# RchalYang/torchrl

Hardware: AMD Instinct MI355X
Metric: env_steps_per_sec_ppo_2048env_halfcheetah_shape (higher is better)
Workload: dtype f32

## Files before the change

torchrl_amd/csrc/k_ppo.hip:

```cpp
#include <cstdlib>
#include "trl_common.h"
#include "trl_mlp.h"
#include "trl_head.h"
#include "trl_comm.h"

struct PpoDev {
  const float *obs, *acts, *advs, *rets, *old_values, *old_logp;
  const int64_t* row_idx;
  int rows_mb, N;
  const double* adv_raw;
  double n_global;
  const float *pf_params, *vf_params;
  float clip_para, entropy_coeff;
  int clipped_value_loss, tanh_action;
  int loss_mode;
  float* partial;
  double* scal_partial;
  int n_wg, n_pf, p_stride;
  int D, A;
};

template <int D, int H, int A> struct PpoShape {
  static_assert(H == 64 && D > 16 && D <= 32 && A <= 8, "instantiated for 16 < D <= 32, H == 64, A <= 8");
  static constexpr int P_PF = MlpFlat<D, H, A>::P_PF, P_VF = MlpFlat<D, H, 1>::P_VF;
  static constexpr int P_STRIDE = ((P_PF > P_VF ? P_PF : P_VF) + 63) & ~63;
};

#define WV_WAVES 4
#ifdef TRL_EXP_CLK
#define WCLK_DECL long long clk_prev = clock64(); float clk_acc[24]; for (int q_ = 0; q_ < 24; ++q_) clk_acc[q_] = 0.f;
#define WCLK(ph) { __builtin_amdgcn_sched_barrier(0); const long long c_ = clock64(); clk_acc[ph] += (float)(c_ - clk_prev); clk_prev = c_; __builtin_amdgcn_sched_barrier(0); }
#else
#define WCLK_DECL
#define WCLK(ph)
#endif
#define WV_THREADS (64 * WV_WAVES)
#define LDT 20
#define LDW 68

template <int D, int H, int A> struct WvShape {
  static_assert(H == 64 && (D == 17 || D == 32) && A <= 8, "instantiated for D == 17 / 32, H == 64, A <= 8");
  static constexpr int O_W2F = 0, O_W2B = H * LDW, O_B1 = 2 * H * LDW, O_B2 = O_B1 + H, O_SCR = O_B2 + H;
  static constexpr int O_H1 = 0, O_H2 = H * LDT, O_DZ2 = 2 * H * LDT, O_DO = 3 * H * LDT, WSCR = O_DO + 16 * LDT;
  static constexpr int P_STRIDE = PpoShape<D, H, A>::P_STRIDE;
  static constexpr int MAIN = O_SCR + WV_WAVES * WSCR;
  static constexpr int XS_W2 = 0, XS_W1 = 16, XS_W1B = 20, XS_W3 = D > 17 ? 24 : 20, XS_PF = XS_W3 + 4, XS_VF = XS_W3;
  static constexpr int XSC_PF = 3 * H + 32, XSC_VF = 4 * H + 16;
  static constexpr int XCH_PF = WV_WAVES * (XS_PF * 256 + XSC_PF), XCH_VF = WV_WAVES * (XS_VF * 256 + XSC_VF);
  static constexpr int XCH = XCH_PF > XCH_VF ? XCH_PF : XCH_VF;
  static constexpr int LDS_FLOATS = MAIN > XCH ? MAIN : XCH;
};

template <int D, int H, int A> struct WvShapeSD : WvShape<D, H, A> {
  static constexpr int P_PF_SD = H * D + H + H * H + H + 2 * A * H + 2 * A, P_VF = MlpFlat<D, H, 1>::P_VF;
  static constexpr int P_STRIDE = ((P_PF_SD > P_VF ? P_PF_SD : P_VF) + 63) & ~63;
};
template <int D, int H, int A, int HEAD> struct WvPick { using T = WvShape<D, H, A>; };
template <int D, int H, int A> struct WvPick<D, H, A, HEAD_SD> { using T = WvShapeSD<D, H, A>; };
#define SD_HALF_LOG_2PI_PLUS_HALF 1.4189385332046727f

__device__ __forceinline__ f32x4 lds4(const float* p) { return *reinterpret_cast<const f32x4*>(p); }
__device__ __forceinline__ float row_sum16(float v) {
  v += __builtin_bit_cast(float, __builtin_amdgcn_update_dpp(0, __builtin_bit_cast(int, v), 0x128, 0xF, 0xF, false));
  v += __builtin_bit_cast(float, __builtin_amdgcn_update_dpp(0, __builtin_bit_cast(int, v), 0x124, 0xF, 0xF, false));
  v += __builtin_bit_cast(float, __builtin_amdgcn_update_dpp(0, __builtin_bit_cast(int, v), 0x122, 0xF, 0xF, false));
  v += __builtin_bit_cast(float, __builtin_amdgcn_update_dpp(0, __builtin_bit_cast(int, v), 0x121, 0xF, 0xF, false));
  return v;
}

template <int D, int H, int A, int ACT, bool IS_PF, bool CONTIG, bool RT, int HEAD = HEAD_GAUSS>
__device__ void ppo_wave_pass(const PpoDev& a, float* lds, int wg_in_net, int n_wg_net) {
  using S = typename WvPick<D, H, A, HEAD>::T;
  constexpr bool WIDE = D > 17,
                 CAT = HEAD == HEAD_CAT, SD = HEAD == HEAD_SD,
                 SDP = SD && IS_PF;
  static_assert(!WIDE || RT, "the wide tile exists as a runtime-dims instantiation only");
  static_assert(!CAT || (IS_PF && RT), "the categorical head is a policy pass of the runtime-dims kernels");
  static_assert(!SD || RT, "the state-dependent-std head belongs to the runtime-dims kernels");
  constexpr int AS = CAT ? 1 : 0;
  const int Dr = RT ? a.D : D;
  const int O = IS_PF ? (RT ? a.A : A) : 1;
  const int OH = SDP ? 2 * O : O;
  const int F_W1 = 0, F_B1 = H * Dr, F_W2 = F_B1 + H, F_B2 = F_W2 + H * H, F_W3 = F_B2 + H, F_B3 = F_W3 + OH * H,
            F_LS = F_B3 + OH, F_END = (CAT || SDP) ? F_LS : F_LS + O;
  auto sd_has = [&](int o) -> bool { return (o & 7) < O; };
  auto sd_row = [&](int o) -> int { return o < 8 ? o : O + (o - 8); };
  const int PS = RT ? a.p_stride : S::P_STRIDE;
  const int tid = threadIdx.x, lane = tid & 63, wave = tid >> 6;
  const int j = lane & 15, g = lane >> 4, i = j;
  const float* gp = IS_PF ? a.pf_params : a.vf_params;
  WCLK_DECL
  float* W2F = lds + S::O_W2F;
  float* W2B = lds + S::O_W2B;
  float* scr = lds + S::O_SCR + wave * S::WSCR;
  float* H1S = scr + S::O_H1;
  float* H2S = scr + S::O_H2;
  float* DZ2S = scr + S::O_DZ2;
  float* DOS = scr + S::O_DO;

  const double adv_s1 = IS_PF ? a.adv_raw[0] : 0.0, adv_s2 = IS_PF ? a.adv_raw[1] : 0.0;
  const int B = a.rows_mb * a.N;
  const int n_tiles = (B + 15) / 16;
  const int tile_stride = n_wg_net * WV_WAVES;

  float xq[5], xtq[4], lq[6];
  float xq2[4], xtq2[4];
  int tile = wg_in_net * WV_WAVES + wave;
  const int tpr = a.N >> 4;
  int p1r = 0, p1c = 0, p2r = 0, p2c = 0, st_r = 0, st_c = 0;
  int64_t ridx1 = 0, ridx2 = 0;
  bool fv[4], fv2[4];
  const bool f16 = !WIDE && (!RT || Dr > 16), jv = !RT || i < Dr, jv2 = WIDE && 16 + i < Dr;
  const unsigned ox16 = (unsigned)(j * Dr + (f16 ? 16 : 0)) * 4u, os = (unsigned)j * 4u;
  unsigned oxq[4], oxt[4], oa_[4], oxq2[4], oxt2[4];
#pragma unroll
  for (int q = 0; q < 4; ++q) {
    fv[q] = !RT || 4 * g + q < Dr;
    fv2[q] = WIDE && 16 + 4 * g + q < Dr;
    oxq[q] = (unsigned)(j * Dr + (fv[q] ? 4 * g + q : 0)) * 4u;
    oxt[q] = (unsigned)((4 * g + q) * Dr + (jv ? i : 0)) * 4u;
    oxq2[q] = (unsigned)(j * Dr + (fv2[q] ? 16 + 4 * g + q : 0)) * 4u;
    oxt2[q] = (unsigned)((4 * g + q) * Dr + (jv2 ? 16 + i : 0)) * 4u;
    if constexpr (SDP) oa_[q] = (unsigned)(j * O + (4 * (g & 1) + q < O ? 4 * (g & 1) + q : 0)) * 4u;
    else oa_[q] = CAT ? (unsigned)j * 4u : (unsigned)(j * O + (4 * g + q < O ? 4 * g + q : 0)) * 4u;
  }
  auto ldb = [](const float* base, unsigned byte_off) -> float {
    return *reinterpret_cast<const float*>(reinterpret_cast<const char*>(base) + byte_off);
  };
  auto pos_advance = [&](int& r, int& c) { c += st_c; r += st_r; if (c >= tpr) { c -= tpr; ++r; } };
  auto load_ridx = [&](int r) -> int64_t {
    const int rr = r < a.rows_mb ? r : 0;
    return a.row_idx ? a.row_idx[rr] : (int64_t)rr;
  };
  auto fetch_contig = [&](int64_t ridx, int r, int c) {
    const int64_t cell0 = (r < a.rows_mb) ? ridx * a.N + 16 * c : 0;
    const float* ob = a.obs + cell0 * Dr;
#pragma unroll
    for (int q = 0; q < 4; ++q) xq[q] = ldb(ob, oxq[q]);
    xq[4] = ldb(ob, ox16);
#pragma unroll
    for (int q = 0; q < 4; ++q) xtq[q] = ldb(ob, oxt[q]);
    if constexpr (WIDE) {
#pragma unroll
      for (int q = 0; q < 4; ++q) { xq2[q] = ldb(ob, oxq2[q]); xtq2[q] = ldb(ob, oxt2[q]); }
    }
    if constexpr (IS_PF) {
      const float* ab = a.acts + cell0 * (CAT ? AS : O);
      if constexpr (CAT) { lq[0] = ldb(ab, oa_[0]); lq[1] = lq[2] = lq[3] = 0.0f; }
      else {
#pragma unroll
        for (int q = 0; q < 4; ++q) lq[q] = ldb(ab, oa_[q]);
      }
      lq[4] = ldb(a.advs + cell0, os);
      lq[5] = a.old_logp ? ldb(a.old_logp + cell0, os) : 0.0f;
    } else {
      lq[0] = lq[1] = lq[2] = lq[3] = 0.0f;
      lq[4] = ldb(a.rets + cell0, os);
      lq[5] = a.clipped_value_loss ? ldb(a.old_values + cell0, os) : 0.0f;
    }
  };
  auto row_of = [&](int smp, int& e) -> int { const int sm = smp < B ? smp : 0; const int r = sm / a.N; e = sm - r * a.N; return r; };
  auto fetch_inputs = [&](int64_t p, int s0) {
#pragma unroll
    for (int r = 0; r < 4; ++r) xq[r] = a.obs[p * Dr + (fv[r] ? 4 * g + r : 0)];
    xq[4] = a.obs[p * Dr + (f16 ? 16 : 0)];
#pragma unroll
    for (int q = 0; q < 4; ++q) {
      const int sj = 4 * g + q;
      const int64_t pr = __shfl(p, sj, 64);
      xtq[q] = a.obs[(s0 + sj < B ? pr : 0) * Dr + (jv ? i : 0)];
      if constexpr (WIDE) {
        xq2[q] = a.obs[p * Dr + (fv2[q] ? 16 + 4 * g + q : 0)];
        xtq2[q] = a.obs[(s0 + sj < B ? pr : 0) * Dr + (jv2 ? 16 + i : 0)];
      }
    }
    if constexpr (IS_PF) {
      if constexpr (CAT) { lq[0] = a.acts[p]; lq[1] = lq[2] = lq[3] = 0.0f; }
      else if constexpr (SDP) {
#pragma unroll
        for (int r = 0; r < 4; ++r) lq[r] = a.acts[p * O + (4 * (g & 1) + r < O ? 4 * (g & 1) + r : 0)];
      } else {
#pragma unroll
        for (int r = 0; r < 4; ++r) lq[r] = a.acts[p * O + (4 * g + r < O ? 4 * g + r : 0)];
      }
      lq[4] = a.advs[p]; lq[5] = a.old_logp ? a.old_logp[p] : 0.0f;
    } else {
      lq[0] = lq[1] = lq[2] = lq[3] = 0.0f;
      lq[4] = a.rets[p]; lq[5] = a.clipped_value_loss ? a.old_values[p] : 0.0f;
    }
  };
  int e_nn = 0;
  int64_t ridx_nn = 0;
  auto fetch_row = [&](int t) {
    const int r = row_of(t * 16 + j, e_nn);
    ridx_nn = a.row_idx ? a.row_idx[r] : (int64_t)r;
  };
  auto prefetch_next = [&](int nt) {
    if constexpr (CONTIG) {
      fetch_contig(ridx1, p1r, p1c);
      p1r = p2r; p1c = p2c; ridx1 = ridx2;
      pos_advance(p2r, p2c);
      ridx2 = load_ridx(p2r);
    } else {
      const int64_t pn = (nt * 16 + j < B) ? ridx_nn * a.N + e_nn : 0;
      fetch_inputs(pn, nt * 16);
      fetch_row(nt + tile_stride);
    }
  };
  if constexpr (CONTIG) {
    const int t0 = __builtin_amdgcn_readfirstlane(tile);
    const int ts = __builtin_amdgcn_readfirstlane(tile_stride);
    st_r = ts / tpr; st_c = ts - st_r * tpr;
    int r0 = t0 / tpr, c0 = t0 - (t0 / tpr) * tpr;
    fetch_contig(load_ridx(r0), r0, c0);
    p1r = r0; p1c = c0;
    pos_advance(p1r, p1c);
    ridx1 = load_ridx(p1r);
    p2r = p1r; p2c = p1c;
    pos_advance(p2r, p2c);
    ridx2 = load_ridx(p2r);
  } else {
    fetch_row(tile);
    const int64_t p0 = (tile * 16 + j < B) ? ridx_nn * a.N + e_nn : 0;
    fetch_inputs(p0, tile * 16);
    fetch_row(tile + tile_stride);
  }
  constexpr int NV = H * H / (4 * WV_THREADS);
  f32x4 wv[NV], wt[NV];
  const int tc = tid & 63, tq = tid >> 6;
  const float bias1 = tid < H ? gp[F_B1 + tid] : 0.0f, bias2 = tid < H ? gp[F_B2 + tid] : 0.0f;
  {
    static_assert(WV_THREADS == 256 && H == 64, "the transposed staging maps (column, 4 rows) onto 256 threads");
    const bool w2_al = !RT || ((reinterpret_cast<uintptr_t>(gp + F_W2) & 15) == 0);
#pragma unroll
    for (int t = 0; t < NV; ++t) {
      if (w2_al) wv[t] = *reinterpret_cast<const f32x4*>(gp + F_W2 + 4 * (tid + WV_THREADS * t));
      else {
#pragma unroll
        for (int x = 0; x < 4; ++x) wv[t][x] = gp[F_W2 + 4 * (tid + WV_THREADS * t) + x];
      }
    }
#pragma unroll
    for (int t = 0; t < NV; ++t)
#pragma unroll
      for (int x = 0; x < 4; ++x) wt[t][x] = gp[F_W2 + (4 * (tq + 4 * t) + x) * H + tc];
  }
  for (int e = lane; e < 16 * LDT; e += 64) DOS[e] = 0.0f;
  float w1[4][5], w3h[4][4], w3t[4][4];
  float w1b[4][4];
#pragma unroll
  for (int so = 0; so < 4; ++so) {
    const int row = 16 * so + i;
#pragma unroll
    for (int r = 0; r < 4; ++r) w1[so][r] = fv[r] ? gp[F_W1 + row * Dr + (fv[r] ? 4 * g + r : 0)] : 0.0f;
    w1[so][4] = (g == 0 && f16) ? gp[F_W1 + row * Dr + (f16 ? 16 : 0)] : 0.0f;
    if constexpr (WIDE) {
#pragma unroll
      for (int r = 0; r < 4; ++r) w1b[so][r] = fv2[r] ? gp[F_W1 + row * Dr + (fv2[r] ? 16 + 4 * g + r : 0)] : 0.0f;
    }
#pragma unroll
    for (int r = 0; r < 4; ++r) {
      if constexpr (SDP) {
        const int o = 4 * g + r;
        w3h[so][r] = sd_has(i) ? gp[F_W3 + (sd_has(i) ? sd_row(i) : 0) * H + 16 * so + 4 * g + r] : 0.0f;
        w3t[so][r] = sd_has(o) ? gp[F_W3 + (sd_has(o) ? sd_row(o) : 0) * H + row] : 0.0f;
      } else if constexpr (IS_PF) {
        w3h[so][r] = (i < O) ? gp[F_W3 + (i < O ? i : 0) * H + 16 * so + 4 * g + r] : 0.0f;
        const int o = 4 * g + r;
        w3t[so][r] = (o < O) ? gp[F_W3 + (o < O ? o : 0) * H + row] : 0.0f;
      } else {
        w3h[so][r] = gp[F_W3 + 16 * so + 4 * g + r];
        w3t[so][r] = 0.0f;
      }
    }
  }
  float lsv[4], ivv[4], b3v[4], lspass[4];
#pragma unroll
  for (int r = 0; r < 4; ++r) {
    const int o = 4 * g + r;
    const float raw = (IS_PF && !CAT && !SDP && o < O) ? gp[F_LS + (o < O ? o : 0)] : 0.0f;
    lsv[r] = fminf(fmaxf(raw, -20.0f), 2.0f);
    ivv[r] = __expf(-2.0f * lsv[r]);
    lspass[r] = (raw >= -20.0f && raw <= 2.0f) ? 1.0f : 0.0f;
    if constexpr (SDP) b3v[r] = sd_has(o) ? gp[F_B3 + (sd_has(o) ? sd_row(o) : 0)] : 0.0f;
    else b3v[r] = (o < O) ? gp[F_B3 + (o < O ? o : 0)] : 0.0f;
  }
  const float vb3 = IS_PF ? 0.0f : gp[F_B3];
#ifdef TRL_EXP_CLK
  WCLK(22)
  __builtin_amdgcn_s_waitcnt(0);
  WCLK(23)
#endif
#pragma unroll
  for (int t = 0; t < NV; ++t) {
    const int e = 4 * (tid + WV_THREADS * t), r = e / H, c = e - r * H;
    *reinterpret_cast<f32x4*>(W2F + r * LDW + c) = wv[t];
    *reinterpret_cast<f32x4*>(W2B + tc * LDW + 4 * (tq + 4 * t)) = wt[t];
  }
  if (tid < H) { lds[S::O_B1 + tid] = bias1; lds[S::O_B2 + tid] = bias2; }
  __syncthreads();

  const double ng = a.n_global;
  const double adv_mean = adv_s1 / ng;
  const double adv_var = (adv_s2 - adv_s1 * adv_s1 / ng) / (ng - 1.0);
  const float adv_mu = (float)adv_mean;
  const float adv_rstd = 1.0f / ((float)sqrt(fmax(adv_var, 0.0)) + 1e-5f);
  const float inv_b = (float)(1.0 / ng);

  f32x4 gW2[4][4], gW1[4], gW3[4];
  f32x4 gW1b[4];
  float gb1[4][4], gb2[4][4], gW1c[4][4];
  float db3[4], dls[4], stv[7];
  float ent_sum = 0.0f;
  float sdst[8] = {0.0f, 0.0f, -INFINITY, -INFINITY, 0.0f, 0.0f, -INFINITY, -INFINITY}, sd_cnt = 0.0f;
#pragma unroll
  for (int x = 0; x < 4; ++x) {
    gW1[x] = gW3[x] = gW1b[x] = f32x4{0.f, 0.f, 0.f, 0.f};
    db3[x] = dls[x] = 0.0f;
#pragma unroll
    for (int y = 0; y < 4; ++y) { gW2[x][y] = f32x4{0.f, 0.f, 0.f, 0.f}; gb1[x][y] = gb2[x][y] = gW1c[x][y] = 0.0f; }
  }
#pragma unroll
  for (int k = 0; k < 7; ++k) stv[k] = (k >= 2 && k <= 5) ? -INFINITY : 0.0f;

  WCLK(0)
  for (; tile < n_tiles; tile += tile_stride) {
    const int s = tile * 16 + j;
    const bool valid = CONTIG ? true : (s < B);
    float xb[5], xt[4], lin[6], xb2[4], xt2[4];
#pragma unroll
    for (int r = 0; r < 4; ++r) xb[r] = (valid && fv[r]) ? xq[r] : 0.0f;
    xb[4] = (valid && f16) ? xq[4] : 0.0f;
#pragma unroll
    for (int q = 0; q < 4; ++q) xt[q] = (jv && (CONTIG || tile * 16 + 4 * g + q < B)) ? xtq[q] : 0.0f;
    if constexpr (WIDE) {
#pragma unroll
      for (int q = 0; q < 4; ++q) {
        xb2[q] = (valid && fv2[q]) ? xq2[q] : 0.0f;
        xt2[q] = (jv2 && (CONTIG || tile * 16 + 4 * g + q < B)) ? xtq2[q] : 0.0f;
      }
    }
#pragma unroll
    for (int q = 0; q < 6; ++q) lin[q] = lq[q];
    const float x16 = xb[4];

#define PIN_DS() __builtin_amdgcn_sched_barrier(0x676)
    f32x4 h1[4], h2[4];
    f32x4 wq[4], bq;
#pragma unroll
    for (int so = 0; so < 4; ++so) h1[so] = lds4(lds + S::O_B1 + 16 * so + 4 * g);
#pragma unroll
    for (int sl = 0; sl < 4; ++sl) wq[sl] = lds4(W2F + i * LDW + 16 * sl + 4 * g);
    bq = lds4(lds + S::O_B2 + 4 * g);
    PIN_DS();
    WCLK(9)
#pragma unroll
    for (int q = 0; q < (WIDE ? 4 : 5); ++q)
#pragma unroll
      for (int so = 0; so < 4; ++so) h1[so] = mfma16(w1[so][q], xb[q], h1[so]);
    if constexpr (WIDE) {
#pragma unroll
      for (int q = 0; q < 4; ++q)
#pragma unroll
        for (int so = 0; so < 4; ++so) h1[so] = mfma16(w1b[so][q], xb2[q], h1[so]);
    }
    WCLK(10)
#pragma unroll
    for (int so = 0; so < 4; ++so)
#pragma unroll
      for (int r = 0; r < 4; ++r) {
        h1[so][r] = act_fn<ACT>(h1[so][r]);
        H1S[(16 * so + 4 * g + r) * LDT + j] = h1[so][r];
      }
    WCLK(1)
#pragma unroll
    for (int so = 0; so < 4; ++so) {
      f32x4 acc = bq;
      f32x4 wc[4];
#pragma unroll
      for (int sl = 0; sl < 4; ++sl) wc[sl] = wq[sl];
      if (so < 3) {
#pragma unroll
        for (int sl = 0; sl < 4; ++sl) wq[sl] = lds4(W2F + (16 * (so + 1) + i) * LDW + 16 * sl + 4 * g);
        bq = lds4(lds + S::O_B2 + 16 * (so + 1) + 4 * g);
        PIN_DS();
      }
#pragma unroll
      for (int sl = 0; sl < 4; ++sl)
#pragma unroll
        for (int r = 0; r < 4; ++r) acc = mfma16(wc[sl][r], h1[sl][r], acc);
      WCLK(11)
#pragma unroll
      for (int r = 0; r < 4; ++r) h2[so][r] = act_fn<ACT>(acc[r]);
      WCLK(12)
    }

    prefetch_next(tile + tile_stride);
    WCLK(2)
    f32x4 dz2[4];
    f32x4 wb[4];
    if constexpr (IS_PF) {
#pragma unroll
      for (int so = 0; so < 4; ++so)
#pragma unroll
        for (int r = 0; r < 4; ++r) H2S[(16 * so + 4 * g + r) * LDT + j] = h2[so][r];
      f32x4 oa = f32x4{b3v[0], b3v[1], b3v[2], b3v[3]}, ob = f32x4{0.f, 0.f, 0.f, 0.f};
#pragma unroll
      for (int sl = 0; sl < 4; sl += 2)
#pragma unroll
        for (int r = 0; r < 4; ++r) { oa = mfma16(w3h[sl][r], h2[sl][r], oa); ob = mfma16(w3h[sl + 1][r], h2[sl + 1][r], ob); }
      WCLK(14)
      float zc[4], lp = 0.0f;
      float pk[4], lpk[4], ent = 0.0f;
      int ai = 0;
      if constexpr (CAT) {
        float lg[4], ek[4], m = -INFINITY;
#pragma unroll
        for (int r = 0; r < 4; ++r) {
          lg[r] = oa[r] + ob[r];
          m = (4 * g + r < O) ? fmaxf(m, lg[r]) : m;
        }
        m = fmaxf(m, __shfl_xor(m, 16, 64));
        m = g < 2 ? m : 0.0f;
#pragma unroll
        for (int r = 0; r < 4; ++r) ek[r] = (4 * g + r < O) ? expf(lg[r] - m) : 0.0f;
        const float c_own = ((ek[0] + ek[1]) + ek[2]) + ek[3];
        const float c_lo = __shfl_xor(c_own, 16, 64);
        float Ssum = g == 1 ? (((c_lo + ek[0]) + ek[1]) + ek[2]) + ek[3] : c_own;
        const float S_hi = __shfl_xor(Ssum, 16, 64);
        Ssum = g == 0 ? S_hi : (g == 1 ? Ssum : 1.0f);
        const float logS = logf(Ssum);
        ai = min(max((int)lin[0], 0), O - 1);
#pragma unroll
        for (int r = 0; r < 4; ++r) {
          const bool has = 4 * g + r < O;
          lpk[r] = has ? (lg[r] - m) - logS : 0.0f;
          pk[r] = ek[r] / Ssum;
          lp += (has && 4 * g + r == ai) ? lpk[r] : 0.0f;
          ent -= pk[r] * lpk[r];
        }
        lp += __shfl_xor(lp, 16, 64);
        ent += __shfl_xor(ent, 16, 64);
      } else if constexpr (SDP) {
#pragma unroll
        for (int r = 0; r < 4; ++r) {
          const bool has = 4 * (g & 1) + r < O;
          const float mine = oa[r] + ob[r], oth = __shfl_xor(mine, 32, 64);
          const float mean = g < 2 ? mine : oth, raw = g < 2 ? oth : mine;
          lsv[r] = fminf(fmaxf(raw, -20.0f), 2.0f);
          ivv[r] = __expf(-2.0f * lsv[r]);
          lspass[r] = (raw >= -20.0f && raw <= 2.0f) ? 1.0f : 0.0f;
          const float t = gauss_logp_term((valid && has) ? lin[r] : 0.0f, has ? mean : 0.0f, ivv[r], lsv[r], a.tanh_action, zc[r]);
          lp += has ? t : 0.0f;
          ent += has ? SD_HALF_LOG_2PI_PLUS_HALF + lsv[r] : 0.0f;
          zc[r] = has ? zc[r] : 0.0f;
        }
        lp += __shfl_xor(lp, 16, 64);
        ent += __shfl_xor(ent, 16, 64);
      } else {
#pragma unroll
      for (int r = 0; r < 4; ++r) {
        const bool has = 4 * g + r < O;
        const float t = gauss_logp_term((valid && has) ? lin[r] : 0.0f, has ? oa[r] + ob[r] : 0.0f, ivv[r], lsv[r],
                                        a.tanh_action, zc[r]);
        lp += has ? t : 0.0f;
        zc[r] = has ? zc[r] : 0.0f;
      }
      WCLK(18)
      lp += __shfl_xor(lp, 16, 64);
      }
      WCLK(19)
      const float advn = valid ? (lin[4] - adv_mu) * adv_rstd : 0.0f;
      float ratio, s1, s2, g_lp;
      if (a.loss_mode == TRL_LOSS_A2C) {
        ratio = 1.0f;
        s1 = s2 = lp * advn;
        g_lp = (valid && (SDP || g < 2)) ? -advn * inv_b : 0.0f;
      } else {
        ratio = __expf(lp - lin[5]);
        s1 = ratio * advn;
        s2 = fminf(fmaxf(ratio, 1.0f - a.clip_para), 1.0f + a.clip_para) * advn;
        g_lp = (valid && (SDP || g < 2) && s1 <= s2) ? -advn * ratio * inv_b : 0.0f;
      }
      WCLK(20)
      float dout[4];
      if constexpr (CAT) {
        const float ce = a.entropy_coeff * inv_b;
#pragma unroll
        for (int r = 0; r < 4; ++r) {
          const bool own = valid && g < 2 && 4 * g + r < O;
          dout[r] = own ? g_lp * ((4 * g + r == ai ? 1.0f : 0.0f) - pk[r]) + ce * pk[r] * (lpk[r] + ent) : 0.0f;
          db3[r] += dout[r];
          if (g < 2) DOS[(4 * g + r) * LDT + j] = dout[r];
        }
        if (valid && g == 0) ent_sum += ent;
      } else if constexpr (SDP) {
        const float ce = a.entropy_coeff * inv_b;
#pragma unroll
        for (int r = 0; r < 4; ++r) {
          const bool own = valid && 4 * (g & 1) + r < O;
          const float dm = g_lp * zc[r] * ivv[r], dr = lspass[r] * (g_lp * (zc[r] * zc[r] * ivv[r] - 1.0f) - ce);
          dout[r] = own ? (g < 2 ? dm : dr) : 0.0f;
          db3[r] += dout[r];
          DOS[(4 * g + r) * LDT + j] = dout[r];
          if (own && g < 2) {
            const float x = lsv[r], ex = expf(x);
            sdst[0] += x; sdst[1] = fmaf(x, x, sdst[1]); sdst[2] = fmaxf(sdst[2], x); sdst[3] = fmaxf(sdst[3], -x);
            sdst[4] += ex; sdst[5] = fmaf(ex, ex, sdst[5]); sdst[6] = fmaxf(sdst[6], ex); sdst[7] = fmaxf(sdst[7], -ex);
          }
        }
        if (valid && g == 0) { ent_sum += ent; sd_cnt += 1.0f; }
      } else {
#pragma unroll
      for (int r = 0; r < 4; ++r) {
        const bool own = valid && g < 2 && 4 * g + r < O;
        dout[r] = own ? g_lp * zc[r] * ivv[r] : 0.0f;
        db3[r] += dout[r];
        dls[r] += own ? lspass[r] * (g_lp * (zc[r] * zc[r] * ivv[r] - 1.0f) - a.entropy_coeff * inv_b) : 0.0f;
        if (g < 2) DOS[(4 * g + r) * LDT + j] = dout[r];
      }
      }
      WCLK(21)
      if (valid && g == 0) {
        stv[0] += lp; stv[1] = fmaf(lp, lp, stv[1]); stv[6] -= fminf(s1, s2);
        stv[2] = fmaxf(stv[2], lp); stv[3] = fmaxf(stv[3], -lp);
        stv[4] = fmaxf(stv[4], ratio); stv[5] = fmaxf(stv[5], -ratio);
      }
      WCLK(15)
      const f32x4 da = lds4(DOS + i * LDT + 4 * g);
      f32x4 hb3[4];
#pragma unroll
      for (int so = 0; so < 4; ++so) hb3[so] = lds4(H2S + (16 * so + j) * LDT + 4 * g);
#pragma unroll
      for (int so = 0; so < 4; ++so) wb[so] = lds4(W2B + (16 * so + i) * LDW + 4 * g);
      PIN_DS();
#pragma unroll
      for (int so = 0; so < 4; ++so) dz2[so] = f32x4{0.f, 0.f, 0.f, 0.f};
#pragma unroll
      for (int r = 0; r < 4; ++r)
#pragma unroll
        for (int so = 0; so < 4; ++so) dz2[so] = mfma16(w3t[so][r], dout[r], dz2[so]);
#pragma unroll
      for (int so = 0; so < 4; ++so)
#pragma unroll
        for (int q = 0; q < 4; ++q) gW3[so] = mfma16(da[q], hb3[so][q], gW3[so]);
      WCLK(16)
    } else {
#pragma unroll
      for (int so = 0; so < 4; ++so) wb[so] = lds4(W2B + (16 * so + i) * LDW + 4 * g);
      PIN_DS();
      float v = 0.0f;
#pragma unroll
      for (int so = 0; so < 4; ++so)
#pragma unroll
        for (int r = 0; r < 4; ++r) v = fmaf(w3h[so][r], h2[so][r], v);
      v += __shfl_xor(v, 16, 64);
      v += __shfl_xor(v, 32, 64);
      v += vb3;
      const float R = lin[4];
      float dv, l;
      if (a.clipped_value_loss) {
        const float vo = lin[5];
        const float dc = v - vo;
        const float vc = vo + fminf(fmaxf(dc, -a.clip_para), a.clip_para);
        const float l1 = (v - R) * (v - R), l2 = (vc - R) * (vc - R);
        const float wa = l1 > l2 ? 1.0f : (l1 == l2 ? 0.5f : 0.0f), wb_ = 1.0f - wa;
        const float pass = (dc >= -a.clip_para && dc <= a.clip_para) ? 1.0f : 0.0f;
        l = 0.5f * fmaxf(l1, l2);
        dv = inv_b * (wa * (v - R) + wb_ * pass * (vc - R));
      } else {
        l = (v - R) * (v - R);
        dv = 2.0f * (v - R) * inv_b;
      }
      dv = valid ? dv : 0.0f;
      if (valid && g == 0) {
        stv[6] += l; db3[0] += dv;
        stv[0] += v; stv[1] = fmaf(v, v, stv[1]); stv[2] = fmaxf(stv[2], v); stv[3] = fmaxf(stv[3], -v);
      }
#pragma unroll
      for (int so = 0; so < 4; ++so)
#pragma unroll
        for (int r = 0; r < 4; ++r) {
          dz2[so][r] = dv * w3h[so][r];
          gW3[so][r] = fmaf(dv, h2[so][r], gW3[so][r]);
        }
    }
#pragma unroll
    for (int so = 0; so < 4; ++so)
#pragma unroll
      for (int r = 0; r < 4; ++r) {
        dz2[so][r] *= act_grad<ACT>(h2[so][r]);
        gb2[so][r] += dz2[so][r];
        DZ2S[(16 * so + 4 * g + r) * LDT + j] = dz2[so][r];
      }

    WCLK(3)
    f32x4 dz1[4];
    f32x4 hb[4], za2;
#pragma unroll
    for (int so = 0; so < 4; ++so) dz1[so] = f32x4{0.f, 0.f, 0.f, 0.f};
#pragma unroll
    for (int sl = 0; sl < 4; ++sl) {
      f32x4 w[4];
// ... 1128 lines not shown
```

Measured before the change: 101.6 million.

## Stage non-W2 parameters through a coalesced LDS image before per-lane gathers

The prologue of the PPO wave pass now loads all parameters except W2 (W1, biases, W3, b3, log-std) cooperatively and coalesced into registers, then writes them to a new LDS image region. Per-lane W1/W3/b3/log-std values are then read from LDS instead of scattered global loads, and the predicate masking is applied after the reads. Input prefetch is moved after the weight loads and fenced with sched_barriers to control issue order. This costs extra LDS per workgroup, which may reduce occupancy, and adds an extra LDS round trip in the prologue.

```diff
diff --git a/torchrl_amd/csrc/k_ppo.hip b/torchrl_amd/csrc/k_ppo.hip
--- a/torchrl_amd/csrc/k_ppo.hip
+++ b/torchrl_amd/csrc/k_ppo.hip
@@ -48,12 +48,18 @@
   static constexpr int XSC_PF = 3 * H + 32, XSC_VF = 4 * H + 16;
   static constexpr int XCH_PF = WV_WAVES * (XS_PF * 256 + XSC_PF), XCH_VF = WV_WAVES * (XS_VF * 256 + XSC_VF);
   static constexpr int XCH = XCH_PF > XCH_VF ? XCH_PF : XCH_VF;
-  static constexpr int LDS_FLOATS = MAIN > XCH ? MAIN : XCH;
+  static constexpr int O_IMG = MAIN > XCH ? MAIN : XCH;
+  static constexpr int IMG_HEAD = 8 * H + 16;
+  static constexpr int IMG = (H * D + 2 * H + IMG_HEAD + WV_THREADS - 1) / WV_THREADS * WV_THREADS;
+  static constexpr int LDS_FLOATS = O_IMG + IMG;
 };
 
 template <int D, int H, int A> struct WvShapeSD : WvShape<D, H, A> {
   static constexpr int P_PF_SD = H * D + H + H * H + H + 2 * A * H + 2 * A, P_VF = MlpFlat<D, H, 1>::P_VF;
   static constexpr int P_STRIDE = ((P_PF_SD > P_VF ? P_PF_SD : P_VF) + 63) & ~63;
+  static constexpr int IMG_HEAD = 16 * H + 16;
+  static constexpr int IMG = (H * D + 2 * H + IMG_HEAD + WV_THREADS - 1) / WV_THREADS * WV_THREADS;
+  static constexpr int LDS_FLOATS = WvShape<D, H, A>::O_IMG + IMG;
 };
 template <int D, int H, int A, int HEAD> struct WvPick { using T = WvShape<D, H, A>; };
 template <int D, int H, int A> struct WvPick<D, H, A, HEAD_SD> { using T = WvShapeSD<D, H, A>; };
@@ -207,12 +213,48 @@
       fetch_row(nt + tile_stride);
     }
   };
+  int r0 = 0, c0 = 0;
+  int64_t ridx0 = 0;
   if constexpr (CONTIG) {
     const int t0 = __builtin_amdgcn_readfirstlane(tile);
     const int ts = __builtin_amdgcn_readfirstlane(tile_stride);
     st_r = ts / tpr; st_c = ts - st_r * tpr;
-    int r0 = t0 / tpr, c0 = t0 - (t0 / tpr) * tpr;
-    fetch_contig(load_ridx(r0), r0, c0);
+    r0 = t0 / tpr; c0 = t0 - (t0 / tpr) * tpr;
+    ridx0 = load_ridx(r0);
+  } else {
+    fetch_row(tile);
+  }
+  __builtin_amdgcn_sched_barrier(0);
+  constexpr int NV = H * H / (4 * WV_THREADS);
+  f32x4 wv[NV], wt[NV];
+  const int tc = tid & 63, tq = tid >> 6;
+  {
+    static_assert(WV_THREADS == 256 && H == 64, "the transposed staging maps (column, 4 rows) onto 256 threads");
+    const bool w2_al = !RT || ((reinterpret_cast<uintptr_t>(gp + F_W2) & 15) == 0);
+#pragma unroll
+    for (int t = 0; t < NV; ++t) {
+      if (w2_al) wv[t] = *reinterpret_cast<const f32x4*>(gp + F_W2 + 4 * (tid + WV_THREADS * t));
+      else {
+#pragma unroll
+        for (int x = 0; x < 4; ++x) wv[t][x] = gp[F_W2 + 4 * (tid + WV_THREADS * t) + x];
+      }
+    }
+#pragma unroll
+    for (int t = 0; t < NV; ++t)
+#pragma unroll
+      for (int x = 0; x < 4; ++x) wt[t][x] = gp[F_W2 + (4 * (tq + 4 * t) + x) * H + tc];
+  }
+  constexpr int NI = S::IMG / WV_THREADS;
+  const int n_img = F_W2 + (F_END - F_B2);
+  float im[NI];
+#pragma unroll
+  for (int k = 0; k < NI; ++k) {
+    const int e = tid + WV_THREADS * k, ec = e < n_img ? e : n_img - 1;
+    im[k] = gp[ec < F_W2 ? ec : ec + H * H];
+  }
+  __builtin_amdgcn_sched_barrier(0);
+  if constexpr (CONTIG) {
+    fetch_contig(ridx0, r0, c0);
     p1r = r0; p1c = c0;
     pos_advance(p1r, p1c);
     ridx1 = load_ridx(p1r);
@@ -220,85 +262,100 @@
     pos_advance(p2r, p2c);
     ridx2 = load_ridx(p2r);
   } else {
-    fetch_row(tile);
     const int64_t p0 = (tile * 16 + j < B) ? ridx_nn * a.N + e_nn : 0;
     fetch_inputs(p0, tile * 16);
     fetch_row(tile + tile_stride);
   }
-  constexpr int NV = H * H / (4 * WV_THREADS);
-  f32x4 wv[NV], wt[NV];
-  const int tc = tid & 63, tq = tid >> 6;
-  const float bias1 = tid < H ? gp[F_B1 + tid] : 0.0f, bias2 = tid < H ? gp[F_B2 + tid] : 0.0f;
-  {
-    static_assert(WV_THREADS == 256 && H == 64, "the transposed staging maps (column, 4 rows) onto 256 threads");
-    const bool w2_al = !RT || ((reinterpret_cast<uintptr_t>(gp + F_W2) & 15) == 0);
-#pragma unroll
-    for (int t = 0; t < NV; ++t) {
-      if (w2_al) wv[t] = *reinterpret_cast<const f32x4*>(gp + F_W2 + 4 * (tid + WV_THREADS * t));
-      else {
-#pragma unroll
-        for (int x = 0; x < 4; ++x) wv[t][x] = gp[F_W2 + 4 * (tid + WV_THREADS * t) + x];
-      }
-    }
-#pragma unroll
-    for (int t = 0; t < NV; ++t)
-#pragma unroll
-      for (int x = 0; x < 4; ++x) wt[t][x] = gp[F_W2 + (4 * (tq + 4 * t) + x) * H + tc];
-  }
-  for (int e = lane; e < 16 * LDT; e += 64) DOS[e] = 0.0f;
-  float w1[4][5], w3h[4][4], w3t[4][4];
-  float w1b[4][4];
-#pragma unroll
-  for (int so = 0; so < 4; ++so) {
-    const int row = 16 * so + i;
-#pragma unroll
-    for (int r = 0; r < 4; ++r) w1[so][r] = fv[r] ? gp[F_W1 + row * Dr + (fv[r] ? 4 * g + r : 0)] : 0.0f;
-    w1[so][4] = (g == 0 && f16) ? gp[F_W1 + row * Dr + (f16 ? 16 : 0)] : 0.0f;
-    if constexpr (WIDE) {
-#pragma unroll
-      for (int r = 0; r < 4; ++r) w1b[so][r] = fv2[r] ? gp[F_W1 + row * Dr + (fv2[r] ? 16 + 4 * g + r : 0)] : 0.0f;
-    }
-#pragma unroll
-    for (int r = 0; r < 4; ++r) {
-      if constexpr (SDP) {
-        const int o = 4 * g + r;
-        w3h[so][r] = sd_has(i) ? gp[F_W3 + (sd_has(i) ? sd_row(i) : 0) * H + 16 * so + 4 * g + r] : 0.0f;
-        w3t[so][r] = sd_has(o) ? gp[F_W3 + (sd_has(o) ? sd_row(o) : 0) * H + row] : 0.0f;
-      } else if constexpr (IS_PF) {
-        w3h[so][r] = (i < O) ? gp[F_W3 + (i < O ? i : 0) * H + 16 * so + 4 * g + r] : 0.0f;
-        const int o = 4 * g + r;
-        w3t[so][r] = (o < O) ? gp[F_W3 + (o < O ? o : 0) * H + row] : 0.0f;
-      } else {
-        w3h[so][r] = gp[F_W3 + 16 * so + 4 * g + r];
-        w3t[so][r] = 0.0f;
-      }
-    }
-  }
-  float lsv[4], ivv[4], b3v[4], lspass[4];
-#pragma unroll
-  for (int r = 0; r < 4; ++r) {
-    const int o = 4 * g + r;
-    const float raw = (IS_PF && !CAT && !SDP && o < O) ? gp[F_LS + (o < O ? o : 0)] : 0.0f;
-    lsv[r] = fminf(fmaxf(raw, -20.0f), 2.0f);
-    ivv[r] = __expf(-2.0f * lsv[r]);
-    lspass[r] = (raw >= -20.0f && raw <= 2.0f) ? 1.0f : 0.0f;
-    if constexpr (SDP) b3v[r] = sd_has(o) ? gp[F_B3 + (sd_has(o) ? sd_row(o) : 0)] : 0.0f;
-    else b3v[r] = (o < O) ? gp[F_B3 + (o < O ? o : 0)] : 0.0f;
-  }
-  const float vb3 = IS_PF ? 0.0f : gp[F_B3];
 #ifdef TRL_EXP_CLK
   WCLK(22)
   __builtin_amdgcn_s_waitcnt(0);
   WCLK(23)
 #endif
+  for (int e = lane; e < 16 * LDT; e += 64) DOS[e] = 0.0f;
 #pragma unroll
   for (int t = 0; t < NV; ++t) {
     const int e = 4 * (tid + WV_THREADS * t), r = e / H, c = e - r * H;
     *reinterpret_cast<f32x4*>(W2F + r * LDW + c) = wv[t];
     *reinterpret_cast<f32x4*>(W2B + tc * LDW + 4 * (tq + 4 * t)) = wt[t];
   }
-  if (tid < H) { lds[S::O_B1 + tid] = bias1; lds[S::O_B2 + tid] = bias2; }
+  float* img = lds + S::O_IMG;
+  constexpr int KB_LO = H * (WIDE ? 18 : RT ? 2 : D) / WV_THREADS, KB_HI = (H * D + 2 * H - 1) / WV_THREADS;
+#pragma unroll
+  for (int k = 0; k < NI; ++k) {
+    const int e = tid + WV_THREADS * k;
+    img[e] = im[k];
+    if (k >= KB_LO && k <= KB_HI && e >= F_B1 && e < F_B1 + 2 * H) lds[S::O_B1 + (e - F_B1)] = im[k];
+  }
+  static_assert(S::O_B2 == S::O_B1 + H, "b1 | b2 are stored as one run");
   __syncthreads();
+
+  const int I_W3 = F_W3 - H * H, I_B3 = F_B3 - H * H, I_LS = F_LS - H * H;
+  float w1[4][5], w3h[4][4], w3t[4][4];
+  float w1b[4][4];
+  float b3v[4], lsraw[4];
+#pragma unroll
+  for (int so = 0; so < 4; ++so) {
+    const int row = 16 * so + i;
+#pragma unroll
+    for (int r = 0; r < 4; ++r) w1[so][r] = img[F_W1 + row * Dr + (fv[r] ? 4 * g + r : 0)];
+    w1[so][4] = img[F_W1 + row * Dr + (f16 ? 16 : 0)];
+    if constexpr (WIDE) {
+#pragma unroll
+      for (int r = 0; r < 4; ++r) w1b[so][r] = img[F_W1 + row * Dr + (fv2[r] ? 16 + 4 * g + r : 0)];
+    }
+#pragma unroll
+    for (int r = 0; r < 4; ++r) {
+      const int o = 4 * g + r;
+      if constexpr (SDP) {
+        w3h[so][r] = img[I_W3 + (sd_has(i) ? sd_row(i) : 0) * H + 16 * so + 4 * g + r];
+        w3t[so][r] = img[I_W3 + (sd_has(o) ? sd_row(o) : 0) * H + row];
+      } else if constexpr (IS_PF) {
+        w3h[so][r] = img[I_W3 + (i < O ? i : 0) * H + 16 * so + 4 * g + r];
+        w3t[so][r] = img[I_W3 + (o < O ? o : 0) * H + row];
+      } else {
+        w3h[so][r] = img[I_W3 + 16 * so + 4 * g + r];
+        w3t[so][r] = 0.0f;
+      }
+    }
+  }
+#pragma unroll
+  for (int r = 0; r < 4; ++r) {
+    const int o = 4 * g + r;
+    if constexpr (IS_PF && !CAT && !SDP) lsraw[r] = img[I_LS + (o < O ? o : 0)];
+    else lsraw[r] = 0.0f;
+    if constexpr (SDP) b3v[r] = img[I_B3 + (sd_has(o) ? sd_row(o) : 0)];
+    else b3v[r] = img[I_B3 + (o < O ? o : 0)];
+  }
+  const float vb3 = IS_PF ? 0.0f : img[I_B3];
+  __builtin_amdgcn_sched_barrier(0);
+#pragma unroll
+  for (int so = 0; so < 4; ++so) {
+#pragma unroll
+    for (int r = 0; r < 4; ++r) {
+      const int o = 4 * g + r;
+      w1[so][r] = fv[r] ? w1[so][r] : 0.0f;
+      if constexpr (WIDE) w1b[so][r] = fv2[r] ? w1b[so][r] : 0.0f;
+      if constexpr (SDP) {
+        w3h[so][r] = sd_has(i) ? w3h[so][r] : 0.0f;
+        w3t[so][r] = sd_has(o) ? w3t[so][r] : 0.0f;
+      } else if constexpr (IS_PF) {
+        w3h[so][r] = (i < O) ? w3h[so][r] : 0.0f;
+        w3t[so][r] = (o < O) ? w3t[so][r] : 0.0f;
+      }
+    }
+    w1[so][4] = (g == 0 && f16) ? w1[so][4] : 0.0f;
+  }
+  float lsv[4], ivv[4], lspass[4];
+#pragma unroll
+  for (int r = 0; r < 4; ++r) {
+    const int o = 4 * g + r;
+    const float raw = (IS_PF && !CAT && !SDP && o < O) ? lsraw[r] : 0.0f;
+    lsv[r] = fminf(fmaxf(raw, -20.0f), 2.0f);
+    ivv[r] = __expf(-2.0f * lsv[r]);
+    lspass[r] = (raw >= -20.0f && raw <= 2.0f) ? 1.0f : 0.0f;
+    if constexpr (SDP) b3v[r] = sd_has(o) ? b3v[r] : 0.0f;
+    else b3v[r] = (o < O) ? b3v[r] : 0.0f;
+  }
 
   const double ng = a.n_global;
   const double adv_mean = adv_s1 / ng;
```

After: 103.0 million, median of 6. 1.01x the previous value.
